# DavidLBick/espnet-1

Hardware: AMD Instinct MI355X
Metric: utterances/sec + step-time, Conformer-L T=1000 batch=32 @1/2/4/8 GPU (higher is better)
Workload: dtype bf16; 1 GPU; C3 Conformer-L (12x512, 8 heads, ff 2048, cnn 31) + 6-layer Transformer decoder, hybrid CTC/att 0.3/0.7, lsm 0.1, V=5000, T=1000 frames x 80, L=40, dropout 0.1, Adam+WarmupLR+clip 5; global_batch=32, seq_len=1000, parallelism=dp1

## Files before the change

espnet-1_amd/csrc/elementwise.hip:

```cpp
#include "common.h"

#include <cstdlib>
#include <cstring>

namespace {

__global__ void mvn_kernel(int B, int T, int F, const float* __restrict__ x, const long long* __restrict__ lens,
                           float* __restrict__ y) {
  const int b = blockIdx.x;
  const int f = threadIdx.x;
  __shared__ double red[1024];
  const long long L = lens[b];
  double s = 0.0;
  const int ty = threadIdx.y, ny = blockDim.y;
  if (f < F)
    for (int t = ty; t < T; t += ny)
      if (t < L) s += x[((long)b * T + t) * F + f];
  red[ty * blockDim.x + f] = s;
  __syncthreads();
  if (ty == 0 && f < F) {
    double a = 0.0;
    for (int k = 0; k < ny; ++k) a += red[k * blockDim.x + f];
    red[f] = a;
  }
// ... 483 lines not shown
    const float wk = w[c * K + k];
#pragma unroll
    for (int j = 0; j < 8; ++j) acc[j] += wk * tile[(tq * 8 + j + k) * DW_CT + cc];
  }
#pragma unroll
  for (int j = 0; j < 8; ++j) {
    const int t = t0 + tq * 8 + j;
    if (t < T) y[((long)b * T + t) * C + c] = acc[j];
  }
}

__global__ __launch_bounds__(256) void dwconv_bwd_kernel(int B, int T, int C, int K, const float* __restrict__ x,
                                                         const float* __restrict__ w, const float* __restrict__ dy,
                                                         float* __restrict__ dx, float* __restrict__ part) {
  extern __shared__ float sm[];
  const int P = (K - 1) / 2;
  const int ntt = ea_cdiv(T, DW_TT);
  const int b = blockIdx.x / ntt, t0 = (blockIdx.x % ntt) * DW_TT;
  const int c0 = blockIdx.y * DW_CT;
  const int rowsL = DW_TT + K - 1;
  float* tdy = sm;
  float* tx = sm + rowsL * DW_CT;
  float* tin = tx + rowsL * DW_CT;
  for (int i = threadIdx.x; i < rowsL * DW_CT; i += blockDim.x) {
    const int rr = i / DW_CT, cc = i % DW_CT, c = c0 + cc;
    const int td = t0 + rr - (K - 1 - P);
    const int tx_ = t0 + rr - P;
    tdy[i] = (td >= 0 && td < T && c < C) ? dy[((long)b * T + td) * C + c] : 0.f;
    tx[i] = (tx_ >= 0 && tx_ < T && c < C) ? x[((long)b * T + tx_) * C + c] : 0.f;
  }
  for (int i = threadIdx.x; i < DW_TT * DW_CT; i += blockDim.x) {
    const int rr = i / DW_CT, cc = i % DW_CT, c = c0 + cc, t = t0 + rr;
    tin[i] = (t < T && c < C) ? dy[((long)b * T + t) * C + c] : 0.f;
  }
  __syncthreads();
  const int cc = threadIdx.x % DW_CT, tq = threadIdx.x / DW_CT;
  const int c = c0 + cc;
  if (c < C) {
    float acc[8];
#pragma unroll
    for (int j = 0; j < 8; ++j) acc[j] = 0.f;
    for (int k = 0; k < K; ++k) {
      const float wk = w[c * K + k];
#pragma unroll
      for (int j = 0; j < 8; ++j) acc[j] += wk * tdy[(tq * 8 + j - k + (K - 1)) * DW_CT + cc];
    }
#pragma unroll
    for (int j = 0; j < 8; ++j) {
      const int t = t0 + tq * 8 + j;
      if (t < T) dx[((long)b * T + t) * C + c] = acc[j];
    }
  }
  const long blk = (long)blockIdx.x;
  if (c < C) {
    for (int k = tq; k < K; k += 4) {
      float a = 0.f;
      for (int r = 0; r < DW_TT; ++r) a += tin[r * DW_CT + cc] * tx[(r + k) * DW_CT + cc];
      part[blk * (long)C * K + (long)c * K + k] = a;
    }
  }
}

constexpr int DW_R = 16;

EA_DEV float4 glu4(const bf16* __restrict__ g2, long row, int C, int c) {
  const uint2 ua = *(const uint2*)(g2 + row * 2 * C + c), ub = *(const uint2*)(g2 + row * 2 * C + C + c);
  const float a0 = __uint_as_float(ua.x << 16), a1 = __uint_as_float(ua.x & 0xffff0000u);
  const float a2 = __uint_as_float(ua.y << 16), a3 = __uint_as_float(ua.y & 0xffff0000u);
  const float b0 = __uint_as_float(ub.x << 16), b1 = __uint_as_float(ub.x & 0xffff0000u);
  const float b2 = __uint_as_float(ub.y << 16), b3 = __uint_as_float(ub.y & 0xffff0000u);
  return make_float4(a0 * sigmoidf_(b0), a1 * sigmoidf_(b1), a2 * sigmoidf_(b2), a3 * sigmoidf_(b3));
}
EA_DEV float glu1(const bf16* __restrict__ g2, long row, int C, int c) {
  return to_f(g2[row * 2 * C + c]) * sigmoidf_(to_f(g2[row * 2 * C + C + c]));
}

template <int K, int R, bool G2IN = false, bool STATS = false>
__global__ __launch_bounds__(256) void dwconv_fwd_k_kernel(int B, int T, int C, const float* __restrict__ x,
                                                           const float* __restrict__ w,
                                                           const float* __restrict__ bias, float* __restrict__ y,
                                                           const bf16* __restrict__ g2 = nullptr,
                                                           float* __restrict__ part = nullptr) {
  constexpr int P = (K - 1) / 2, TT = 4 * R, RL = TT + K - 1, WIN = R + K - 1;
  __shared__ float tile[RL * DW_CT];
  __shared__ float wsm[K * DW_CT];
  const int ntt = ea_cdiv(T, TT);
  const int b = blockIdx.x / ntt, t0 = (blockIdx.x % ntt) * TT;
  const int c0 = blockIdx.y * DW_CT;
  const int cc = threadIdx.x % DW_CT, tq = threadIdx.x / DW_CT;
  const int c = c0 + cc;
  for (int i = threadIdx.x; i < DW_CT * K; i += 256) {
    const int ci = i / K, k = i - ci * K;
    wsm[k * DW_CT + ci] = c0 + ci < C ? w[(long)c0 * K + i] : 0.f;
  }
  if (C % 4 == 0) {
    constexpr int NL = (RL * (DW_CT / 4) + 255) / 256;
    float4 v[NL];
#pragma unroll
    for (int u = 0; u < NL; ++u) {
      const int i = threadIdx.x + 256 * u;
      const int rr = i / (DW_CT / 4), c4 = (i % (DW_CT / 4)) * 4;
      const int t = t0 + rr - P;
      v[u] = make_float4(0.f, 0.f, 0.f, 0.f);
      if (i < RL * (DW_CT / 4) && t >= 0 && t < T && c0 + c4 < C) {
        if constexpr (G2IN)
          v[u] = glu4(g2, (long)b * T + t, C, c0 + c4);
        else
          v[u] = *(const float4*)(x + ((long)b * T + t) * C + c0 + c4);
      }
    }
#pragma unroll
    for (int u = 0; u < NL; ++u) {
      const int i = threadIdx.x + 256 * u;
      if (i < RL * (DW_CT / 4)) *(float4*)(tile + (i / (DW_CT / 4)) * DW_CT + (i % (DW_CT / 4)) * 4) = v[u];
    }
  } else {
    for (int rr = tq; rr < RL; rr += 4) {
      const int t = t0 + rr - P;
      float v = 0.f;
      if (t >= 0 && t < T && c < C) {
        if constexpr (G2IN)
          v = glu1(g2, (long)b * T + t, C, c);
        else
          v = x[((long)b * T + t) * C + c];
      }
      tile[rr * DW_CT + cc] = v;
    }
  }
  __syncthreads();
  if (!STATS && c >= C) return;
  float win[WIN];
#pragma unroll
  for (int i = 0; i < WIN; ++i) win[i] = tile[(tq * R + i) * DW_CT + cc];
  float acc[R];
  const float b0 = bias && c < C ? bias[c] : 0.f;
#pragma unroll
  for (int j = 0; j < R; ++j) acc[j] = b0;
#pragma unroll
  for (int k = 0; k < K; ++k) {
    const float wk = wsm[k * DW_CT + cc];
#pragma unroll
    for (int j = 0; j < R; ++j) acc[j] += wk * win[j + k];
  }
  float s1 = 0.f, s2 = 0.f;
#pragma unroll
  for (int j = 0; j < R; ++j) {
    const int t = t0 + tq * R + j;
    if (t < T && c < C) {
      y[((long)b * T + t) * C + c] = acc[j];
      if constexpr (STATS) {
        const float d = acc[j] - b0;
        s1 += d;
        s2 += d * d;
      }
    }
  }
  if constexpr (STATS) {
    __shared__ float red[2][4][DW_CT];
    red[0][tq][cc] = s1;
    red[1][tq][cc] = s2;
    __syncthreads();
    if (tq == 0 && c < C) {
      part[(long)blockIdx.x * 2 * C + c] = (red[0][0][cc] + red[0][1][cc]) + (red[0][2][cc] + red[0][3][cc]);
      part[(long)blockIdx.x * 2 * C + C + c] = (red[1][0][cc] + red[1][1][cc]) + (red[1][2][cc] + red[1][3][cc]);
    }
  }
}

template <int K, int R, bool CK = false, bool GLU = false, bool G2IN = false>
__global__ __launch_bounds__(256) void dwconv_bwd_k_kernel(int B, int T, int C, const float* __restrict__ x,
                                                           const float* __restrict__ w, const float* __restrict__ dy,
                                                           float* __restrict__ dx, float* __restrict__ part,
                                                           const bf16* __restrict__ g2 = nullptr,
                                                           bf16* __restrict__ dg2 = nullptr) {
  constexpr int P = (K - 1) / 2, TT = 4 * R, RL = TT + K - 1, WIN = R + K - 1;
  constexpr int SM = 2 * RL * DW_CT > 4 * (K + 1) * DW_CT ? 2 * RL * DW_CT : 4 * (K + 1) * DW_CT;
  __shared__ float sm[SM];
  float* tdy = sm;
  float* tx = sm + RL * DW_CT;
  const int ntt = ea_cdiv(T, TT);
  const int b = blockIdx.x / ntt, t0 = (blockIdx.x % ntt) * TT;
  const int c0 = blockIdx.y * DW_CT;
  const int cc = threadIdx.x % DW_CT, tq = threadIdx.x / DW_CT;
  const int c = c0 + cc;
  float wr[K];
#pragma unroll
  for (int k = 0; k < K; ++k) wr[k] = c < C ? w[(long)c * K + k] : 0.f;
  bf16 ga[GLU ? R : 1], gb[GLU ? R : 1];
  if constexpr (GLU) {
#pragma unroll
    for (int j = 0; j < R; ++j) {
      const long row = (long)b * T + min(t0 + tq * R + j, T - 1);
      const int cl = min(c, C - 1);
      ga[j] = g2[row * 2 * C + cl];
      gb[j] = g2[row * 2 * C + C + cl];
    }
  }
  if (C % 4 == 0) {
    constexpr int NL = (RL * (DW_CT / 4) + 255) / 256;
    float4 va[NL], vb[NL];
#pragma unroll
    for (int u = 0; u < NL; ++u) {
      const int i = threadIdx.x + 256 * u;
      const int rr = i / (DW_CT / 4), c4 = (i % (DW_CT / 4)) * 4;
      const int td = t0 + rr - (K - 1 - P), tx_ = t0 + rr - P;
      const bool okc = i < RL * (DW_CT / 4) && c0 + c4 < C;
      va[u] = make_float4(0.f, 0.f, 0.f, 0.f);
      vb[u] = va[u];
      if (okc && td >= 0 && td < T) va[u] = *(const float4*)(dy + ((long)b * T + td) * C + c0 + c4);
      if (okc && tx_ >= 0 && tx_ < T) {
        if constexpr (G2IN)
          vb[u] = glu4(g2, (long)b * T + tx_, C, c0 + c4);
        else
          vb[u] = *(const float4*)(x + ((long)b * T + tx_) * C + c0 + c4);
      }
    }
#pragma unroll
    for (int u = 0; u < NL; ++u) {
      const int i = threadIdx.x + 256 * u;
      if (i < RL * (DW_CT / 4)) {
        const int o = (i / (DW_CT / 4)) * DW_CT + (i % (DW_CT / 4)) * 4;
        *(float4*)(tdy + o) = va[u];
        *(float4*)(tx + o) = vb[u];
      }
    }
  } else {
    for (int rr = tq; rr < RL; rr += 4) {
      const int td = t0 + rr - (K - 1 - P), tx_ = t0 + rr - P;
      const bool okc = c < C;
      tdy[rr * DW_CT + cc] = (okc && td >= 0 && td < T) ? dy[((long)b * T + td) * C + c] : 0.f;
      float xv = 0.f;
      if (okc && tx_ >= 0 && tx_ < T) {
        if constexpr (G2IN)
          xv = glu1(g2, (long)b * T + tx_, C, c);
        else
          xv = x[((long)b * T + tx_) * C + c];
      }
      tx[rr * DW_CT + cc] = xv;
    }
  }
  __syncthreads();
  float aw[K + 1];
  {
    float win[WIN];
#pragma unroll
    for (int i = 0; i < WIN; ++i) win[i] = tdy[(tq * R + i) * DW_CT + cc];
    if (c < C) {
      float acc[R];
#pragma unroll
      for (int j = 0; j < R; ++j) acc[j] = 0.f;
#pragma unroll
      for (int k = 0; k < K; ++k) {
        const float wk = wr[k];
#pragma unroll
        for (int j = 0; j < R; ++j) acc[j] += wk * win[j - k + K - 1];
      }
      if constexpr (GLU) {
#pragma unroll
        for (int j = 0; j < R; ++j) {
          const int t = t0 + tq * R + j;
          if (t < T) {
            const long row = (long)b * T + t;
            const float a = to_f(ga[j]), g = to_f(gb[j]);
            const float s = sigmoidf_(g), d = acc[j];
            dg2[row * 2 * C + c] = from_f<bf16>(d * s);
            dg2[row * 2 * C + C + c] = from_f<bf16>(d * a * s * (1.f - s));
          }
        }
      } else {
#pragma unroll
        for (int j = 0; j < R; ++j) {
          const int t = t0 + tq * R + j;
          if (t < T) dx[((long)b * T + t) * C + c] = acc[j];
        }
      }
    }
    float xw[WIN];
#pragma unroll
    for (int i = 0; i < WIN; ++i) xw[i] = tx[(tq * R + i) * DW_CT + cc];
#pragma unroll
    for (int k = 0; k <= K; ++k) aw[k] = 0.f;
#pragma unroll
    for (int j = 0; j < R; ++j) {
      const float d = win[j + K - 1 - P];
      aw[K] += d;
#pragma unroll
      for (int k = 0; k < K; ++k) aw[k] += d * xw[j + k];
    }
  }
  __syncthreads();
#pragma unroll
  for (int k = 0; k <= K; ++k) sm[(tq * (K + 1) + k) * DW_CT + cc] = aw[k];
  __syncthreads();
  const long blk = (long)blockIdx.x;
  for (int i = threadIdx.x; i < (K + 1) * DW_CT; i += blockDim.x) {
    const int k = CK ? (i < K * DW_CT ? i % K : K) : i / DW_CT;
    const int ci = CK ? (i < K * DW_CT ? i / K : i - K * DW_CT) : i % DW_CT;
    const int cg = c0 + ci;
    if (cg >= C) continue;
    const float v = (sm[(0 * (K + 1) + k) * DW_CT + ci] + sm[(1 * (K + 1) + k) * DW_CT + ci]) +
                    (sm[(2 * (K + 1) + k) * DW_CT + ci] + sm[(3 * (K + 1) + k) * DW_CT + ci]);
    const long o = CK ? (k < K ? (long)cg * K + k : (long)C * K + cg) : (long)k * C + cg;
    part[blk * (long)C * (K + 1) + o] = v;
  }
}

template <typename T>
__global__ void add_pos_bias_kernel(long N, int H, int dk, const T* __restrict__ q, long ldq, const float* __restrict__ u,
                                    const float* __restrict__ v, T* __restrict__ qu, T* __restrict__ qv) {
  const int d = H * dk;
  const long n = N * d;
  for (long i = blockIdx.x * (long)blockDim.x + threadIdx.x; i < n; i += (long)gridDim.x * blockDim.x) {
    const long r = i / d;
    const int c = (int)(i % d);
    const float x = to_f(q[r * ldq + c]);
    qu[i] = from_f<T>(x + u[c]);
    qv[i] = from_f<T>(x + v[c]);
  }
}

__global__ void embed_fwd_kernel(long rows, int d, int L, const long long* __restrict__ tok, const float* __restrict__ E,
                                 float xscale, const float* __restrict__ pe, float p, uint64_t seed,
                                 const unsigned long long* salt, float* __restrict__ y) {
  if (p > 0.f) seed = ea_salted(seed, salt);
  const long n = rows * d;
  for (long i = blockIdx.x * (long)blockDim.x + threadIdx.x; i < n; i += (long)gridDim.x * blockDim.x) {
    const long r = i / d;
    const int c = (int)(i % d);
    float v = E[tok[r] * d + c] * xscale + pe[(r % L) * d + c];
    if (p > 0.f) v *= drop_scale(seed, (uint64_t)i, p);
    y[i] = v;
  }
}
__global__ void add_pe_dropout_kernel(long n, int d, int L, const float* __restrict__ pe, float p, uint64_t seed,
                                      const unsigned long long* salt, float* __restrict__ y) {
  if (p > 0.f) seed = ea_salted(seed, salt);
  for (long i = blockIdx.x * (long)blockDim.x + threadIdx.x; i < n; i += (long)gridDim.x * blockDim.x) {
    const long r = i / d;
    const int c = (int)(i % d);
    float v = y[i] + pe[(r % L) * d + c];
    if (p > 0.f) v *= drop_scale(seed, (uint64_t)i, p);
    y[i] = v;
  }
}
constexpr int EMBED_BWD_MAXROWS = 4096;
__global__ __launch_bounds__(256) void embed_bwd_kernel(int rows, int d, const long long* __restrict__ tok,
                                                        const float* __restrict__ dy, float xscale, float p,
                                                        uint64_t seed, const unsigned long long* salt,
                                                        float* __restrict__ dE) {
  __shared__ int stok[EMBED_BWD_MAXROWS];
  __shared__ int dup;
  if (p > 0.f) seed = ea_salted(seed, salt);
  const int r = blockIdx.x;
  const long long me = tok[r];
  if (threadIdx.x == 0) dup = 0;
  __syncthreads();
  for (int q = threadIdx.x; q < rows; q += blockDim.x) {
    stok[q] = (int)tok[q];
    if (q < r && tok[q] == me) dup = 1;
  }
  __syncthreads();
  if (dup) return;
  __shared__ int list[EMBED_BWD_MAXROWS];
  __shared__ int wcnt[4], nlist;
  const int lane = threadIdx.x & 63, w = threadIdx.x >> 6;
  if (threadIdx.x == 0) nlist = 0;
  __syncthreads();
  for (int base = r; base < rows; base += 256) {
    const int q = base + threadIdx.x;
    const bool hit = q < rows && stok[q] == (int)me;
    const unsigned long long m = __ballot(hit);
    if (lane == 0) wcnt[w] = __popcll(m);
    __syncthreads();
    int off = nlist;
    for (int v = 0; v < w; ++v) off += wcnt[v];
    if (hit) list[off + __popcll(m & ((1ull << lane) - 1ull))] = q;
    __syncthreads();
    if (threadIdx.x == 0) nlist += wcnt[0] + wcnt[1] + wcnt[2] + wcnt[3];
    __syncthreads();
  }
  const int n = nlist;
  for (int c = threadIdx.x; c < d; c += blockDim.x) {
    float a = 0.f;
    for (int k = 0; k < n; ++k) {
      const int q = list[k];
      const uint64_t i = (uint64_t)q * d + c;
      float v = dy[i] * xscale;
      if (p > 0.f) v *= drop_scale(seed, i, p);
      a += v;
    }
    dE[me * d + c] += a;
  }
}

__global__ void argmax_rows_kernel(long rows, int V, const float* __restrict__ x, long ld, long long* __restrict__ out) {
  const int lane = threadIdx.x & 63;
  const long r = blockIdx.x * (long)(blockDim.x >> 6) + (threadIdx.x >> 6);
  if (r >= rows) return;
  const float* xr = x + r * ld;
  float best = -INFINITY;
  int bi = 0x7fffffff;
  for (int v = lane; v < V; v += 64) {
    const float t = xr[v];
    if (t > best || (t == best && v < bi) || (t != t && best == best)) { best = t; bi = v; }
  }
#pragma unroll
  for (int o = 32; o > 0; o >>= 1) {
    const float ob = __shfl_xor(best, o, 64);
    const int oi = __shfl_xor(bi, o, 64);
    const bool on = ob != ob, bn = best != best;
    if (on ? (!bn || oi < bi) : (!bn && (ob > best || (ob == best && oi < bi)))) { best = ob; bi = oi; }
  }
  if (lane == 0) out[r] = bi;
}

}

#define EA_GRID(n) dim3(ea_grid_cap(ea_cdiv((n), 256))), dim3(256), 0, (hipStream_t)stream

extern "C" int ea_utterance_mvn(int B, int T, int F, const float* x, const long long* lens, float* y, void* stream) {
  EA_ENTRY();
  EA_CHECK_ARG(F <= 256 && F > 0);
  const int bx = F <= 64 ? 64 : (F <= 128 ? 128 : 256);
  const int by = 1024 / bx;
  hipLaunchKernelGGL(mvn_kernel, dim3(B), dim3(bx, by), 0, (hipStream_t)stream, B, T, F, x, lens, y);
  EA_LAUNCH_CHECK();
  return 0;
}

extern "C" int ea_utterance_mvn_ws_bytes(int B, int T, int F, long* bytes) {
  EA_ENTRY();
  EA_CHECK_ARG(bytes != nullptr && B >= 0 && T >= 0 && F > 0);
  *bytes = (long)B * ea_cdiv(T, MVN_TC) * F * (long)sizeof(double);
  return 0;
}

extern "C" int ea_utterance_mvn2(int B, int T, int F, const float* x, const long long* lens, float* y, void* ws,
                                 long ws_bytes, void* stream) {
  EA_ENTRY();
  EA_CHECK_ARG(F <= 256 && F > 0 && ws != nullptr);
  const int nch = ea_cdiv(T, MVN_TC);
  EA_CHECK_ARG(ws_bytes >= (long)B * nch * F * (long)sizeof(double));
  if (B == 0 || T == 0) return 0;
  const int bx = F <= 64 ? 64 : (F <= 128 ? 128 : 256);
  const int by = 512 / bx;
  hipStream_t st = (hipStream_t)stream;
  hipLaunchKernelGGL(mvn_part_kernel, dim3(nch, B), dim3(bx, by), 0, st, T, F, x, lens, (double*)ws);
  EA_LAUNCH_CHECK();
  hipLaunchKernelGGL(mvn_apply_kernel, dim3(nch, B), dim3(bx, by), 0, st, T, F, x, lens, (const double*)ws, y);
  EA_LAUNCH_CHECK();
  return 0;
}

extern "C" int ea_subsample_lens(int B, int T, const long long* ilens, long long* olens, void* stream) {
  EA_ENTRY();
  hipLaunchKernelGGL(subsample_lens_kernel, dim3(ea_cdiv(B, 64)), dim3(64), 0, (hipStream_t)stream, B, T, ilens, olens);
  EA_LAUNCH_CHECK();
  return 0;
}

extern "C" int ea_add_sos_eos(int B, int L, const long long* ys, long ldys, const long long* ylens, int sos, int eos,
                              int ignore_id, long long* ys_in, long long* ys_out, long long* ys_in_lens, void* stream) {
  EA_ENTRY();
  hipLaunchKernelGGL(sos_eos_kernel, dim3(B), dim3(64), 0, (hipStream_t)stream, B, L, ys, ldys, ylens, sos, eos,
                     ignore_id, ys_in, ys_out, ys_in_lens);
  EA_LAUNCH_CHECK();
  return 0;
}

const unsigned long long* ea_g_rng_salt = nullptr;

namespace {
__global__ void rng_advance_kernel(unsigned long long* salt) { salt[0] += 1ull; }
}

extern "C" int ea_set_rng_salt(const unsigned long long* salt) {
  EA_ENTRY();
  ea_g_rng_salt = salt;
  return 0;
}

extern "C" int ea_rng_advance(unsigned long long* salt, void* stream) {
  EA_ENTRY();
  EA_CHECK_ARG(salt != nullptr);
  hipLaunchKernelGGL(rng_advance_kernel, dim3(1), dim3(1), 0, (hipStream_t)stream, salt);
  EA_LAUNCH_CHECK();
  return 0;
}

extern "C" int ea_scale_dropout(long rows, int cols, const void* x, int x_dtype, long ldx, void* y, int y_dtype,
                                long ldy, float scale, float p, unsigned long long seed, void* stream) {
  EA_ENTRY();
  const long n = rows * cols;
  if (n == 0) return 0;
  const int xa = x_dtype == EA_BF16 ? 8 : 16, ya = y_dtype == EA_BF16 ? 8 : 16;
  if (cols % 4 == 0 && ldx % 4 == 0 && ldy % 4 == 0 && (uintptr_t)x % xa == 0 && (uintptr_t)y % ya == 0 &&
      n / 4 < (1L << 31)) {
    const unsigned n4 = (unsigned)(n / 4), c4 = (unsigned)(cols / 4);
#define EA_SDV(TI, TO) hipLaunchKernelGGL((scale_drop_vec_kernel<TI, TO>), EA_GRID(n4), n4, c4, (const TI*)x, ldx, (TO*)y, ldy, scale, p, (uint64_t)seed, ea_g_rng_salt)
    if (x_dtype == EA_BF16 && y_dtype == EA_BF16) EA_SDV(bf16, bf16);
    else if (x_dtype == EA_BF16) EA_SDV(bf16, float);
    else if (y_dtype == EA_BF16) EA_SDV(float, bf16);
    else EA_SDV(float, float);
#undef EA_SDV
    EA_LAUNCH_CHECK();
    return 0;
  }
#define EA_SD(TI, TO) hipLaunchKernelGGL((scale_drop_kernel<TI, TO>), EA_GRID(n), n, cols, (const TI*)x, ldx, (TO*)y, ldy, scale, p, (uint64_t)seed, ea_g_rng_salt)
  if (x_dtype == EA_BF16 && y_dtype == EA_BF16) EA_SD(bf16, bf16);
  else if (x_dtype == EA_BF16) EA_SD(bf16, float);
  else if (y_dtype == EA_BF16) EA_SD(float, bf16);
  else EA_SD(float, float);
#undef EA_SD
  EA_LAUNCH_CHECK();
  return 0;
}

extern "C" int ea_add_2d(long rows, int cols, const void* x, int x_dtype, long ldx, void* y, int y_dtype,
                          long ldy, float alpha, void* stream) {
  EA_ENTRY();
  const long n = rows * cols;
  if (n == 0) return 0;
  const int xa = x_dtype == EA_BF16 ? 8 : 16, ya = y_dtype == EA_BF16 ? 8 : 16;
  if (cols % 4 == 0 && ldx % 4 == 0 && ldy % 4 == 0 && (uintptr_t)x % xa == 0 && (uintptr_t)y % ya == 0 &&
      n / 4 < (1L << 31)) {
    const unsigned n4 = (unsigned)(n / 4), c4 = (unsigned)(cols / 4);
#define EA_A2V(TI, TO) hipLaunchKernelGGL((add2d_vec_kernel<TI, TO>), EA_GRID(n4), n4, c4, (const TI*)x, ldx, (TO*)y, ldy, alpha)
    if (x_dtype == EA_BF16 && y_dtype == EA_BF16) EA_A2V(bf16, bf16);
    else if (x_dtype == EA_BF16) EA_A2V(bf16, float);
    else if (y_dtype == EA_BF16) EA_A2V(float, bf16);
    else EA_A2V(float, float);
#undef EA_A2V
    EA_LAUNCH_CHECK();
    return 0;
  }
#define EA_A2(TI, TO) hipLaunchKernelGGL((add2d_kernel<TI, TO>), EA_GRID(n), n, cols, (const TI*)x, ldx, (TO*)y, ldy, alpha)
  if (x_dtype == EA_BF16 && y_dtype == EA_BF16) EA_A2(bf16, bf16);
  else if (x_dtype == EA_BF16) EA_A2(bf16, float);
  else if (y_dtype == EA_BF16) EA_A2(float, bf16);
  else EA_A2(float, float);
#undef EA_A2
  EA_LAUNCH_CHECK();
  return 0;
}

extern "C" int ea_permute3(int A, int Bd, int Cd, const void* src, int src_dtype, void* dst, int dst_dtype,
                           int accumulate, void* stream) {
  EA_ENTRY();
  const long n = (long)A * Bd * Cd;
  if (n == 0) return 0;
#define EA_P3(TI, TO) hipLaunchKernelGGL((permute3_kernel<TI, TO>), EA_GRID(n), A, Bd, Cd, (const TI*)src, (TO*)dst, accumulate)
  if (src_dtype == EA_BF16 && dst_dtype == EA_BF16) EA_P3(bf16, bf16);
  else if (src_dtype == EA_BF16) EA_P3(bf16, float);
  else if (dst_dtype == EA_BF16) EA_P3(float, bf16);
  else EA_P3(float, float);
#undef EA_P3
  EA_LAUNCH_CHECK();
  return 0;
}

extern "C" int ea_im2col_conv1(int B, int T, int F, const float* x, void* col, int col_dtype, void* stream) {
  EA_ENTRY();
  const int T1 = (T - 3) / 2 + 1, F1 = (F - 3) / 2 + 1;
  const long n = (long)B * T1 * F1 * 16;
  if (col_dtype == EA_BF16)
    hipLaunchKernelGGL(im2col_conv1_kernel<bf16>, EA_GRID(n), B, T, F, T1, F1, x, (bf16*)col);
  else
    hipLaunchKernelGGL(im2col_conv1_kernel<float>, EA_GRID(n), B, T, F, T1, F1, x, (float*)col);
  EA_LAUNCH_CHECK();
  return 0;
}

extern "C" int ea_im2col_conv2(int B, int T1, int F1, int C, const void* x1, void* col, int dtype, void* stream) {
  EA_ENTRY();
  EA_CHECK_ARG(C % 8 == 0);
  const int T2 = (T1 - 3) / 2 + 1, F2 = (F1 - 3) / 2 + 1;
  const long n = (long)B * T2 * F2 * 9 * (C / 8);
  if (dtype == EA_BF16)
    hipLaunchKernelGGL(im2col_conv2_kernel<bf16>, EA_GRID(n), B, T1, F1, C, T2, F2, (const bf16*)x1, (bf16*)col);
  else
    hipLaunchKernelGGL(im2col_conv2_kernel<float>, EA_GRID(n), B, T1, F1, C, T2, F2, (const float*)x1, (float*)col);
  EA_LAUNCH_CHECK();
  return 0;
}

extern "C" int ea_col2im_conv2(int B, int T1, int F1, int C, const void* dcol, int dcol_dtype, const void* x1,
                               void* dx1, int dtype, void* stream) {
  EA_ENTRY();
  const int T2 = (T1 - 3) / 2 + 1, F2 = (F1 - 3) / 2 + 1;
  const long n = (long)B * T1 * F1 * C;
  if (dcol_dtype == EA_BF16 && dtype == EA_BF16 && C % 8 == 0) {
    hipLaunchKernelGGL(col2im_conv2_bf16x8_kernel, EA_GRID(n / 8), B, T1, F1, C, T2, F2, (const bf16*)dcol,
                       (const bf16*)x1, (bf16*)dx1);
    EA_LAUNCH_CHECK();
    return 0;
  }
#define EA_C2I(TI, TO) hipLaunchKernelGGL((col2im_conv2_kernel<TI, TO>), EA_GRID(n), B, T1, F1, C, T2, F2, (const TI*)dcol, (const TO*)x1, (TO*)dx1)
  if (dcol_dtype == EA_BF16 && dtype == EA_BF16) EA_C2I(bf16, bf16);
  else if (dcol_dtype == EA_BF16) EA_C2I(bf16, float);
  else if (dtype == EA_BF16) EA_C2I(float, bf16);
  else EA_C2I(float, float);
#undef EA_C2I
  EA_LAUNCH_CHECK();
  return 0;
}

extern "C" int ea_glu_fwd(long rows, int C, const void* x, int x_dtype, void* y, int y_dtype, void* stream) {
  EA_ENTRY();
  const long n = rows * C;
#define EA_G(TI, TO) hipLaunchKernelGGL((glu_fwd_kernel<TI, TO>), EA_GRID(n), rows, C, (const TI*)x, (TO*)y)
  if (x_dtype == EA_BF16 && y_dtype == EA_BF16) EA_G(bf16, bf16);
  else if (x_dtype == EA_BF16) EA_G(bf16, float);
  else if (y_dtype == EA_BF16) EA_G(float, bf16);
  else EA_G(float, float);
#undef EA_G
  EA_LAUNCH_CHECK();
  return 0;
}

extern "C" int ea_glu_bwd(long rows, int C, const void* x, int x_dtype, const float* dy, void* dx, void* stream) {
  EA_ENTRY();
  const long n = rows * C;
  if (x_dtype == EA_BF16)
    hipLaunchKernelGGL((glu_bwd_kernel<bf16, bf16>), EA_GRID(n), rows, C, (const bf16*)x, dy, (bf16*)dx);
  else
    hipLaunchKernelGGL((glu_bwd_kernel<float, float>), EA_GRID(n), rows, C, (const float*)x, dy, (float*)dx);
  EA_LAUNCH_CHECK();
  return 0;
}

extern "C" int ea_dwconv_fwd(int B, int T, int C, int K, const float* x, const float* w, const float* bias, float* y,
                             void* stream) {
  EA_ENTRY();
  EA_CHECK_ARG(K % 2 == 1);
  dim3 grid(B * ea_cdiv(T, DW_TT), ea_cdiv(C, DW_CT));
  dim3 gridr(B * ea_cdiv(T, 4 * DW_R), ea_cdiv(C, DW_CT));
  hipStream_t st = (hipStream_t)stream;
  switch (K) {
#define EA_DWF(KK) case KK: hipLaunchKernelGGL((dwconv_fwd_k_kernel<KK, DW_R>), gridr, dim3(256), 0, st, B, T, C, x, w, bias, y); break;
    EA_DWF(3) EA_DWF(5) EA_DWF(7) EA_DWF(15) EA_DWF(31)
#undef EA_DWF
    default: {
      const size_t sm = (size_t)(DW_TT + K - 1) * DW_CT * sizeof(float);
      hipLaunchKernelGGL(dwconv_fwd_kernel, grid, dim3(256), sm, st, B, T, C, K, x, w, bias, y);
    }
  }
  EA_LAUNCH_CHECK();
  return 0;
}

extern "C" int ea_dwconv_bwd(int B, int T, int C, int K, const float* x, const float* w, const float* dy, float* dx,
                             float* dw, float* dbias, int accumulate_params, float* workspace, long ws_elems,
                             void* stream) {
  EA_ENTRY();
  EA_CHECK_ARG(K % 2 == 1);
  const int nblk = B * ea_cdiv(T, DW_TT);
  dim3 grid(nblk, ea_cdiv(C, DW_CT));
  if (K == 3 || K == 5 || K == 7 || K == 15 || K == 31) {
    const int nblkr = B * ea_cdiv(T, 4 * DW_R);
    dim3 gridr(nblkr, ea_cdiv(C, DW_CT));
    const long rowlen = (long)C * (K + 1);
    EA_CHECK_ARG((long)nblkr * rowlen <= ws_elems);
    hipStream_t st = (hipStream_t)stream;
    switch (K) {
#define EA_DWB(KK) case KK: hipLaunchKernelGGL((dwconv_bwd_k_kernel<KK, DW_R>), gridr, dim3(256), 0, st, B, T, C, x, w, dy, dx, workspace); break;
      EA_DWB(3) EA_DWB(5) EA_DWB(7) EA_DWB(15) EA_DWB(31)
#undef EA_DWB
    }
    EA_LAUNCH_CHECK();
    int rc = ea_reduce_partials_tr(nblkr, C * K, workspace, rowlen, dw, accumulate_params, C, K, stream);
    if (rc || !dbias) return rc;
    return ea_reduce_partials(nblkr, C, workspace + (long)C * K, rowlen, dbias, accumulate_params, stream);
  }
  EA_CHECK_ARG((long)nblk * C * K <= ws_elems);
  const size_t sm = (size_t)(2 * (DW_TT + K - 1) + DW_TT) * DW_CT * sizeof(float);
  hipStream_t st = (hipStream_t)stream;
  hipLaunchKernelGGL(dwconv_bwd_kernel, grid, dim3(256), sm, st, B, T, C, K, x, w, dy, dx, workspace);
  EA_LAUNCH_CHECK();
  int rc = ea_reduce_partials(nblk, C * K, workspace, (long)C * K, dw, accumulate_params, stream);
  if (rc) return rc;
  if (dbias) return ea_colsum(B * T, C, dy, EA_F32, C, dbias, accumulate_params, workspace, ws_elems, stream);
  return 0;
}

extern "C" int ea_dwconv_fwd_glu(int B, int T, int C, int K, const void* g2, const float* w, const float* bias,
                                 float* y, void* stream) {
  EA_ENTRY();
  EA_CHECK_ARG((K == 3 || K == 5 || K == 7 || K == 15 || K == 31) && g2 && y && C % 4 == 0 &&
               ((uintptr_t)g2 % 8) == 0);
  dim3 gridr(B * ea_cdiv(T, 4 * DW_R), ea_cdiv(C, DW_CT));
  hipStream_t st = (hipStream_t)stream;
  switch (K) {
#define EA_DWF(KK)                                                                                          \
  case KK:                                                                                                  \
    hipLaunchKernelGGL((dwconv_fwd_k_kernel<KK, DW_R, true>), gridr, dim3(256), 0, st, B, T, C, (const float*)nullptr, \
                       w, bias, y, (const bf16*)g2);                                                        \
    break;
    EA_DWF(3) EA_DWF(5) EA_DWF(7) EA_DWF(15) EA_DWF(31)
#undef EA_DWF
  }
  EA_LAUNCH_CHECK();
  return 0;
}

extern "C" int ea_dwconv_fwd_glu_stats(int B, int T, int C, int K, const void* g2, const float* w, const float* bias,
                                       float* y, float* part, void* stream) {
  EA_ENTRY();
  EA_CHECK_ARG((K == 3 || K == 5 || K == 7 || K == 15 || K == 31) && g2 && y && part && bias && C % 4 == 0 &&
               ((uintptr_t)g2 % 8) == 0);
  dim3 gridr(B * ea_cdiv(T, 4 * DW_R), ea_cdiv(C, DW_CT));
  hipStream_t st = (hipStream_t)stream;
  switch (K) {
#define EA_DWF(KK)                                                                                            \
  case KK:                                                                                                    \
    hipLaunchKernelGGL((dwconv_fwd_k_kernel<KK, DW_R, true, true>), gridr, dim3(256), 0, st, B, T, C,           \
                       (const float*)nullptr, w, bias, y, (const bf16*)g2, part);                             \
    break;
    EA_DWF(3) EA_DWF(5) EA_DWF(7) EA_DWF(15) EA_DWF(31)
#undef EA_DWF
  }
  EA_LAUNCH_CHECK();
  return 0;
}

extern "C" int ea_dwconv_stats_parts(int B, int T, int* nparts) {
  EA_ENTRY();
  EA_CHECK_ARG(nparts != nullptr && B > 0 && T > 0);
  *nparts = B * ea_cdiv(T, 4 * DW_R);
  return 0;
}

extern "C" int ea_dwconv_glu_bwd(int B, int T, int C, int K, const float* x, const float* w, const float* dy,
                                 const void* g2, void* dg2, float* dw, float* dbias, int accumulate_params,
                                 float* workspace, long ws_elems, void* stream) {
  EA_ENTRY();
  EA_CHECK_ARG((K == 3 || K == 5 || K == 7 || K == 15 || K == 31) && g2 && dg2 && dw && dbias);
  EA_CHECK_ARG(x != nullptr || (C % 4 == 0 && ((uintptr_t)g2 % 8) == 0));
  const int nblkr = B * ea_cdiv(T, 4 * DW_R);
  dim3 gridr(nblkr, ea_cdiv(C, DW_CT));
  const long rowlen = (long)C * (K + 1);
  EA_CHECK_ARG((long)nblkr * rowlen <= ws_elems);
  hipStream_t st = (hipStream_t)stream;
  const bool adj = dbias == dw + (long)C * K;
  switch (K) {
#define EA_DWB(KK)                                                                                              \
  case KK:                                                                                                      \
    if (x)                                                                                                      \
      hipLaunchKernelGGL((dwconv_bwd_k_kernel<KK, DW_R, false, true>), gridr, dim3(256), 0, st, B, T, C, x, w, dy,   \
                         (float*)nullptr, workspace, (const bf16*)g2, (bf16*)dg2);                                    \
    else                                                                                                        \
      hipLaunchKernelGGL((dwconv_bwd_k_kernel<KK, DW_R, false, true, true>), gridr, dim3(256), 0, st, B, T, C,      \
                         (const float*)nullptr, w, dy, (float*)nullptr, workspace, (const bf16*)g2, (bf16*)dg2);      \
    break;
    EA_DWB(3) EA_DWB(5) EA_DWB(7) EA_DWB(15) EA_DWB(31)
#undef EA_DWB
  }
  EA_LAUNCH_CHECK();
  if (adj) return ea_reduce_partials_tr(nblkr, (int)rowlen, workspace, rowlen, dw, accumulate_params, C, K, stream);
  int rc = ea_reduce_partials_tr(nblkr, C * K, workspace, rowlen, dw, accumulate_params, C, K, stream);
  if (rc) return rc;
  return ea_reduce_partials(nblkr, C, workspace + (long)C * K, rowlen, dbias, accumulate_params, stream);
}


extern "C" int ea_add_pos_bias(long N, int H, int dk, const void* q, long ldq, const float* u, const float* v,
                               void* qu, void* qv, int dtype, void* stream) {
  EA_ENTRY();
  const long n = N * H * dk;
  if (dtype == EA_BF16)
    hipLaunchKernelGGL(add_pos_bias_kernel<bf16>, EA_GRID(n), N, H, dk, (const bf16*)q, ldq, u, v, (bf16*)qu, (bf16*)qv);
  else
    hipLaunchKernelGGL(add_pos_bias_kernel<float>, EA_GRID(n), N, H, dk, (const float*)q, ldq, u, v, (float*)qu, (float*)qv);
  EA_LAUNCH_CHECK();
  return 0;
}

extern "C" int ea_embed_fwd(long rows, int d, int L, const long long* tok, const float* E, float xscale,
                            const float* pe, float p, unsigned long long seed, float* y, void* stream) {
  EA_ENTRY();
  const long n = rows * d;
  hipLaunchKernelGGL(embed_fwd_kernel, EA_GRID(n), rows, d, L, tok, E, xscale, pe, p, (uint64_t)seed, ea_g_rng_salt, y);
  EA_LAUNCH_CHECK();
  return 0;
}

extern "C" int ea_add_pe_dropout(long rows, int d, int L, const float* pe, float p, unsigned long long seed,
                                 float* y, void* stream) {
  EA_ENTRY();
  EA_CHECK_ARG(rows >= 0 && d > 0 && L > 0);
  const long n = rows * d;
  if (n == 0) return 0;
  hipLaunchKernelGGL(add_pe_dropout_kernel, EA_GRID(n), n, d, L, pe, p, (uint64_t)seed, ea_g_rng_salt, y);
  EA_LAUNCH_CHECK();
  return 0;
}

extern "C" int ea_embed_bwd(long rows, int d, const long long* tok, const float* dy, float xscale, float p,
                            unsigned long long seed, float* dE, void* stream) {
  EA_ENTRY();
  EA_CHECK_ARG(rows >= 0 && rows <= EMBED_BWD_MAXROWS);
  if (rows == 0) return 0;
  hipLaunchKernelGGL(embed_bwd_kernel, dim3((unsigned)rows), dim3(256), 0, (hipStream_t)stream, (int)rows, d, tok,
                     dy, xscale, p, (uint64_t)seed, ea_g_rng_salt, dE);
  EA_LAUNCH_CHECK();
  return 0;
}

extern "C" int ea_argmax_rows(long rows, int V, const float* x, long ld, long long* out, void* stream) {
  EA_ENTRY();
  hipLaunchKernelGGL(argmax_rows_kernel, dim3(ea_cdiv(rows, 4)), dim3(256), 0, (hipStream_t)stream, rows, V, x, ld, out);
  EA_LAUNCH_CHECK();
  return 0;
}

static PhaseGeo phase_geo(int B, int T1, int F1, int C) {
  PhaseGeo g;
  g.T1 = T1; g.F1 = F1;
  g.nI0 = (T1 + 1) / 2; g.nI1 = T1 / 2; g.nJ0 = (F1 + 1) / 2; g.nJ1 = F1 / 2;
  g.plane[0] = 0;
  g.plane[1] = (long)B * g.nI0 * g.nJ0;
  g.plane[2] = g.plane[1] + (long)B * g.nI0 * g.nJ1;
  g.plane[3] = g.plane[2] + (long)B * g.nI1 * g.nJ0;
  return g;
}

extern "C" int ea_conv1_fwd2(int B, int T, int F, int C, const float* x, const float* w, const float* bias,
                             void* x1p, int dtype, unsigned char* pos, void* stream) {
  EA_ENTRY();
  EA_CHECK_ARG(C % 8 == 0 && 256 % (C / 8) == 0 && T >= 3 && F >= 3);
  const int T1 = (T - 3) / 2 + 1, F1 = (F - 3) / 2 + 1;
  const PhaseGeo g = phase_geo(B, T1, F1, C);
  const long npix = (long)B * T1 * F1;
  if ((C == 512 || C == 1024 || C == 2048) && (long)B * T1 < (1L << 31)) {
    static int resident = 0;
    if (!resident) {
      int per_cu = 0, dev = 0, ncu = 0;
      (void)hipGetDevice(&dev);
      (void)hipDeviceGetAttribute(&ncu, hipDeviceAttributeMultiprocessorCount, dev);
      (void)hipOccupancyMaxActiveBlocksPerMultiprocessor(&per_cu, conv1_fwd_rows_kernel<bf16, true>, 256, 0);
      resident = std::max(1, per_cu) * std::max(1, ncu);
    }
    dim3 grid((unsigned)std::min<long>((long)B * T1, resident));
    if (dtype == EA_BF16)
      hipLaunchKernelGGL((conv1_fwd_rows_kernel<bf16, true>), grid, dim3(256), 0, (hipStream_t)stream, B, T, F, g, C,
                         x, w, bias, (bf16*)x1p, pos);
    else
      hipLaunchKernelGGL((conv1_fwd_rows_kernel<float, false>), grid, dim3(256), 0, (hipStream_t)stream, B, T, F, g, C, x, w,
                         bias, (float*)x1p, pos);
    EA_LAUNCH_CHECK();
    return 0;
  }
  const int ppb = 256 / (C / 8);
  dim3 grid(ea_grid_cap(ea_cdiv(npix, ppb), 4096));
  if (dtype == EA_BF16)
    hipLaunchKernelGGL(conv1_fwd_kernel<bf16>, grid, dim3(256), 0, (hipStream_t)stream, B, T, F, g, C, x, w, bias,
                       (bf16*)x1p, pos);
  else
    hipLaunchKernelGGL(conv1_fwd_kernel<float>, grid, dim3(256), 0, (hipStream_t)stream, B, T, F, g, C, x, w, bias,
                       (float*)x1p, pos);
  EA_LAUNCH_CHECK();
  return 0;
}

extern "C" int ea_conv1_fwd(int B, int T, int F, int C, const float* x, const float* w, const float* bias,
                            void* x1p, int dtype, void* stream) {
  return ea_conv1_fwd2(B, T, F, C, x, w, bias, x1p, dtype, nullptr, stream);
}

extern "C" int ea_conv1_wgrad(int B, int T, int F, int C, const float* x, const void* dh, int dtype, float* dw,
                              float* dbias, float* workspace, long ws_elems, void* stream) {
  EA_ENTRY();
  EA_CHECK_ARG(C % 8 == 0 && 256 % (C / 8) == 0 && T >= 3 && F >= 3);
  const int T1 = (T - 3) / 2 + 1, F1 = (F - 3) / 2 + 1;
  const PhaseGeo g = phase_geo(B, T1, F1, C);
  const long npix = (long)B * T1 * F1;
  const int ppb = 256 / (C / 8);
  int nb = ea_grid_cap(ea_cdiv(npix, ppb * 16), 1024);
  if ((long)nb > ws_elems / (10L * C)) nb = (int)(ws_elems / (10L * C));
  EA_CHECK_ARG(nb >= 1);
  hipStream_t st = (hipStream_t)stream;
  if (dtype == EA_BF16)
    hipLaunchKernelGGL(conv1_wgrad_kernel<bf16>, dim3(nb), dim3(256), 0, st, B, T, F, g, C, x, (const bf16*)dh, workspace);
  else
    hipLaunchKernelGGL(conv1_wgrad_kernel<float>, dim3(nb), dim3(256), 0, st, B, T, F, g, C, x, (const float*)dh,
                       workspace);
  EA_LAUNCH_CHECK();
  int rc = ea_reduce_partials_tr(nb, 9 * C, workspace, 10L * C, dw, 1, C, 9, stream);
  if (rc) return rc;
  return ea_reduce_partials(nb, C, workspace + 9L * C, 10L * C, dbias, 1, stream);
}

extern "C" int ea_conv1_wgrad_reduce(int ntiles, int C, const float* part, float* dw, float* dbias, void* stream) {
  EA_ENTRY();
  EA_CHECK_ARG(ntiles >= 1 && C >= 1 && part && dw && dbias);
  int rc = ea_reduce_partials_tr(ntiles, 9 * C, part, 10L * C, dw, 1, C, 9, stream);
  if (rc) return rc;
  return ea_reduce_partials(ntiles, C, part + 9L * C, 10L * C, dbias, 1, stream);
}

namespace {
__global__ void relu_inplace_kernel(long n, float* __restrict__ x) {
  for (long i = blockIdx.x * (long)blockDim.x + threadIdx.x; i < n / 4; i += (long)gridDim.x * blockDim.x) {
    float4 v = ((float4*)x)[i];
    v.x = fmaxf(v.x, 0.f); v.y = fmaxf(v.y, 0.f); v.z = fmaxf(v.z, 0.f); v.w = fmaxf(v.w, 0.f);
    ((float4*)x)[i] = v;
  }
  for (long i = (n / 4) * 4 + blockIdx.x * (long)blockDim.x + threadIdx.x; i < n; i += (long)gridDim.x * blockDim.x)
    x[i] = fmaxf(x[i], 0.f);
}
}

extern "C" int ea_relu_f32_inplace(long n, float* x, void* stream) {
  EA_ENTRY();
  EA_CHECK_ARG(n >= 0 && (n == 0 || (x && (uintptr_t)x % 16 == 0)));
  if (n == 0) return 0;
  hipLaunchKernelGGL(relu_inplace_kernel, dim3(ea_grid_cap(ea_cdiv(n / 4 + 1, 256), 4096)), dim3(256), 0,
                     (hipStream_t)stream, n, x);
  EA_LAUNCH_CHECK();
  return 0;
}
```

Measured before the change: 1887 utterances/s.

## Add streaming GLU+depthwise-conv forward kernel with LDS ring buffer and prefetch

```diff
diff --git a/espnet-1_amd/csrc/elementwise.hip b/espnet-1_amd/csrc/elementwise.hip
--- a/espnet-1_amd/csrc/elementwise.hip
+++ b/espnet-1_amd/csrc/elementwise.hip
@@ -809,6 +809,122 @@
                     (sm[(2 * (K + 1) + k) * DW_CT + ci] + sm[(3 * (K + 1) + k) * DW_CT + ci]);
     const long o = CK ? (k < K ? (long)cg * K + k : (long)C * K + cg) : (long)k * C + cg;
     part[blk * (long)C * (K + 1) + o] = v;
+  }
+}
+
+constexpr int DWS_CT = 32, DWS_R = 8, DWS_TT = 64, DWS_RING = 2 * DWS_TT;
+static_assert((256 / DWS_CT) * DWS_R == DWS_TT, "256 threads: 32 channels x 8 row groups of 8 rows");
+EA_DEV float bf_lo(unsigned u) { return __uint_as_float(u << 16); }
+EA_DEV float bf_hi(unsigned u) { return __uint_as_float(u & 0xffff0000u); }
+EA_DEV void dws_load_g2(int T, int C, int b, int row0, int c0, const bf16* __restrict__ g2, uint4& ra, uint4& rb) {
+  const int u = min(max(row0 + (int)threadIdx.x / 4, 0), T - 1), c = min(c0 + ((int)threadIdx.x % 4) * 8, C - 8);
+  const bf16* pa = g2 + (long)b * T * 2 * C;
+  const unsigned o = (unsigned)u * 2u * C + c;
+  ra = *(const uint4*)(pa + o);
+  rb = *(const uint4*)(pa + C + o);
+}
+EA_DEV bool dws_live_g2(int T, int C, int row0, int c0) {
+  const int u = row0 + (int)threadIdx.x / 4;
+  return u >= 0 && u < T && c0 + ((int)threadIdx.x % 4) * 8 < C;
+}
+template <typename TE, unsigned NB>
+EA_DEV TE dws_ring(const void* ring, unsigned a, unsigned off) {
+  return *(const TE*)((const unsigned char*)ring + ((a + off) & (NB - 1u)));
+}
+
+template <int K, bool STATS>
+__global__ __launch_bounds__(256) void dwconv_fwd_stream_kernel(int B, int T, int C, int nseg, int spp,
+                                                                const bf16* __restrict__ g2,
+                                                                const float* __restrict__ w,
+                                                                const float* __restrict__ bias, float* __restrict__ y,
+                                                                float* __restrict__ part) {
+  constexpr int P = (K - 1) / 2, R = DWS_R, CT = DWS_CT, NTQ = 256 / CT, WIN = R + K - 1;
+  constexpr unsigned RB = DWS_RING * CT * 4;
+  static_assert(2 * P <= DWS_TT, "a step's window spans two chunks");
+  __shared__ __attribute__((aligned(16))) float ring[DWS_RING * CT];
+  __shared__ __attribute__((aligned(16))) float outt[DWS_TT * CT];
+  __shared__ float wsm[K * CT];
+  __shared__ float red[STATS ? 2 * NTQ * CT : 1];
+  const int nst = ea_cdiv(T, DWS_TT);
+  const int b = blockIdx.x / nseg, s0 = (blockIdx.x % nseg) * spp, s1 = min(s0 + spp, nst);
+  const int c0 = blockIdx.y * CT;
+  const int cc = threadIdx.x % CT, tq = threadIdx.x / CT;
+  const int c = c0 + cc;
+  for (int i = threadIdx.x; i < CT * K; i += 256) {
+    const int ci = i / K, k = i - ci * K;
+    wsm[k * CT + ci] = c0 + ci < C ? w[(long)c0 * K + i] : 0.f;
+  }
+  const float b0 = bias && c < C ? bias[c] : 0.f;
+  uint4 ra, rb;
+  auto commit = [&](int j) {
+    float4 lo = make_float4(0.f, 0.f, 0.f, 0.f), hi = lo;
+    if (dws_live_g2(T, C, DWS_TT * j + P - DWS_TT, c0)) {
+      lo = make_float4(bf_lo(ra.x) * sigmoidf_(bf_lo(rb.x)), bf_hi(ra.x) * sigmoidf_(bf_hi(rb.x)),
+                       bf_lo(ra.y) * sigmoidf_(bf_lo(rb.y)), bf_hi(ra.y) * sigmoidf_(bf_hi(rb.y)));
+      hi = make_float4(bf_lo(ra.z) * sigmoidf_(bf_lo(rb.z)), bf_hi(ra.z) * sigmoidf_(bf_hi(rb.z)),
+                       bf_lo(ra.w) * sigmoidf_(bf_lo(rb.w)), bf_hi(ra.w) * sigmoidf_(bf_hi(rb.w)));
+    }
+    float* o = ring + ((j & 1) * DWS_TT + threadIdx.x / 4) * CT + (threadIdx.x % 4) * 8;
+    *(float4*)o = lo;
+    *(float4*)(o + 4) = hi;
+  };
+  dws_load_g2(T, C, b, DWS_TT * s0 + P - DWS_TT, c0, g2, ra, rb);
+  commit(s0);
+  dws_load_g2(T, C, b, DWS_TT * (s0 + 1) + P - DWS_TT, c0, g2, ra, rb);
+  for (int s = s0; s < s1; ++s) {
+    const int t0 = DWS_TT * s;
+    commit(s + 1);
+    __syncthreads();
+    if (s + 1 < s1)
+      dws_load_g2(T, C, b, DWS_TT * (s + 2) + P - DWS_TT, c0, g2, ra, rb);
+    const unsigned a0 = (unsigned)((t0 + tq * R + DWS_TT - 2 * P) * CT + cc) * 4u;
+    float win[WIN];
+#pragma unroll
+    for (int i = 0; i < WIN; ++i) win[i] = dws_ring<float, RB>(ring, a0, i * CT * 4);
+    float acc[R];
+#pragma unroll
+    for (int j = 0; j < R; ++j) acc[j] = b0;
+#pragma unroll
+    for (int k = 0; k < K; ++k) {
+      const float wk = wsm[k * CT + cc];
+#pragma unroll
+      for (int j = 0; j < R; ++j) acc[j] += wk * win[j + k];
+    }
+    float s1_ = 0.f, s2_ = 0.f;
+#pragma unroll
+    for (int j = 0; j < R; ++j) {
+      outt[(tq * R + j) * CT + cc] = acc[j];
+      if constexpr (STATS) {
+        if (t0 + tq * R + j < T && c < C) {
+          const float d = acc[j] - b0;
+          s1_ += d;
+          s2_ += d * d;
+        }
+      }
+    }
+    if constexpr (STATS) {
+      red[tq * CT + cc] = s1_;
+      red[(NTQ + tq) * CT + cc] = s2_;
+    }
+    __syncthreads();
+#pragma unroll
+    for (int u = 0; u < DWS_TT * (CT / 4) / 256; ++u) {
+      const int i = threadIdx.x + 256 * u;
+      const int rr = i / (CT / 4), c4 = (i % (CT / 4)) * 4;
+      if (t0 + rr < T && c0 + c4 < C)
+        *(float4*)(y + ((long)b * T + t0 + rr) * C + c0 + c4) = *(const float4*)(outt + rr * CT + c4);
+    }
+    if constexpr (STATS) {
+      if (tq == 0 && c < C) {
+        const float* r1 = red + cc;
+        const float* r2 = red + NTQ * CT + cc;
+        const long row = (long)b * nst + s;
+        part[row * 2 * C + c] = ((r1[0] + r1[CT]) + (r1[2 * CT] + r1[3 * CT])) +
+                                ((r1[4 * CT] + r1[5 * CT]) + (r1[6 * CT] + r1[7 * CT]));
+        part[row * 2 * C + C + c] = ((r2[0] + r2[CT]) + (r2[2 * CT] + r2[3 * CT])) +
+                                    ((r2[4 * CT] + r2[5 * CT]) + (r2[6 * CT] + r2[7 * CT]));
+      }
+    }
   }
 }
 
@@ -1190,6 +1306,38 @@
   return 0;
 }
 
+static bool dw_stream_on(int C, const void* p0, const void* p1, const void* p2) {
+  const char* e = getenv("EA_DWCONV_STREAM");
+  if (e && atoi(e) <= 0) return false;
+  return C % 8 == 0 && C >= 8 && (((uintptr_t)p0 | (uintptr_t)p1 | (uintptr_t)p2) % 16) == 0;
+}
+static void dw_stream_grid(int B, int T, int C, int* nseg, int* spp) {
+  const int nst = ea_cdiv(T, DWS_TT), ncg = ea_cdiv(C, DWS_CT);
+  const char* e = getenv("EA_DWCONV_SPP");
+  int s = e ? atoi(e) : 0;
+  if (s < 1) {
+    const int want = (int)std::min<long>(nst, std::max<long>(1, ea_cdiv(1024, (long)B * ncg)));
+    s = ea_cdiv(nst, want);
+  }
+  *spp = std::min(s, nst);
+  *nseg = ea_cdiv(nst, *spp);
+}
+template <bool STATS>
+static void dw_fwd_stream_launch(int B, int T, int C, int K, const bf16* g2, const float* w, const float* bias,
+                                 float* y, float* part, hipStream_t st) {
+  int nseg, spp;
+  dw_stream_grid(B, T, C, &nseg, &spp);
+  dim3 grid(B * nseg, ea_cdiv(C, DWS_CT));
+  switch (K) {
+#define EA_DWF(KK)                                                                                              \
+  case KK:                                                                                                      \
+    hipLaunchKernelGGL((dwconv_fwd_stream_kernel<KK, STATS>), grid, dim3(256), 0, st, B, T, C, nseg, spp, g2, w, \
+                       bias, y, part);                                                                          \
+    break;
+    EA_DWF(3) EA_DWF(5) EA_DWF(7) EA_DWF(15) EA_DWF(31)
+#undef EA_DWF
+  }
+}
 extern "C" int ea_dwconv_fwd_glu(int B, int T, int C, int K, const void* g2, const float* w, const float* bias,
                                  float* y, void* stream) {
   EA_ENTRY();
@@ -1197,6 +1345,11 @@
                ((uintptr_t)g2 % 8) == 0);
   dim3 gridr(B * ea_cdiv(T, 4 * DW_R), ea_cdiv(C, DW_CT));
   hipStream_t st = (hipStream_t)stream;
+  if (B > 0 && T > 0 && dw_stream_on(C, g2, y, nullptr)) {
+    dw_fwd_stream_launch<false>(B, T, C, K, (const bf16*)g2, w, bias, y, nullptr, st);
+    EA_LAUNCH_CHECK();
+    return 0;
+  }
   switch (K) {
 #define EA_DWF(KK)                                                                                          \
   case KK:                                                                                                  \
@@ -1217,6 +1370,11 @@
                ((uintptr_t)g2 % 8) == 0);
   dim3 gridr(B * ea_cdiv(T, 4 * DW_R), ea_cdiv(C, DW_CT));
   hipStream_t st = (hipStream_t)stream;
+  if (B > 0 && T > 0 && dw_stream_on(C, g2, y, nullptr)) {
+    dw_fwd_stream_launch<true>(B, T, C, K, (const bf16*)g2, w, bias, y, part, st);
+    EA_LAUNCH_CHECK();
+    return 0;
+  }
   switch (K) {
 #define EA_DWF(KK)                                                                                            \
   case KK:                                                                                                    \
@@ -1250,7 +1408,7 @@
   hipStream_t st = (hipStream_t)stream;
   const bool adj = dbias == dw + (long)C * K;
   switch (K) {
-#define EA_DWB(KK)                                                                                              \
+#define EA_DWB(KK)                                                                                           \
   case KK:                                                                                                      \
     if (x)                                                                                                      \
       hipLaunchKernelGGL((dwconv_bwd_k_kernel<KK, DW_R, false, true>), gridr, dim3(256), 0, st, B, T, C, x, w, dy,   \
```

After: 1886 utterances/s (median of 3 runs). No clear change (-0.0%).
